# sqeazy/sqeazy

Measured on AMD Instinct MI355X. Metric: encode GB/s (input voxels) for bitswap1->lz4 uint16 volume, higher is better.
Workload: dtype u16

## Files before the change

### sqeazy_amd/csrc/sqy_capi.cpp

```cpp
#include "../../include/sqeazy_amd.h"

#include <hip/hip_runtime.h>

#include <algorithm>
#include <chrono>
#include <climits>
#include <cstdint>
#include <cstdio>
#include <cstdlib>
#include <cstring>
#include <atomic>
#include <condition_variable>
#include <memory>
#include <mutex>
#include <string>
#include <thread>
#include <vector>

#include "sqy_kernels.h"
#include "sqy_lanes.hpp"
#include "sqy_pipeline.hpp"

namespace {

// ... 558 lines not shown
    int produced(const uint8_t* out) { cur = out; return 0; }
    bool is_tail(size_t si) const { return pipe.sink_index >= 0 && (int)si > pipe.sink_index; }
    bool not_3d(const char* scheme) const
    {
        if (dims.size() != 3) std::fprintf(stderr, "[sqeazy::detail::%s::encode] received non-3D shape which is currently unsupported!\n", scheme);
        return dims.size() != 3;
    }
    bool followed_by(size_t si, StageKind k) const { return si + 1 < pipe.stages.size() && pipe.stages[si + 1].kind == k; }
    void stage_shape(size_t si, uint64_t& Z, uint64_t& Y, uint64_t& X) const
    {
        const bool flat = is_tail(si) && cur_len * (uint64_t)cur_elem != len;
        Z = flat ? 1 : dims[0]; Y = flat ? 1 : dims[1]; X = flat ? cur_len : dims[2];
    }

    int take_lanes(std::unique_lock<std::mutex>& lock)
    {
        const long mode = g_opt.stage_lanes.load();
        if (!lanes || mode == 0 || (mode == 2 && !g_opt.transpose_chain_caller_streams.load()) || (stream != nullptr && stream == cx.stream)) return 0;
        int devid = 0;
        if (hipGetDevice(&devid) != hipSuccess || devid < 0 || devid >= kMaxDev) return 0;
        if (!cx.ensure_lane_event()) { std::fprintf(stderr, "[sqeazy]\t no HIP event for the lanes\n"); return 1; }
        const auto deadline = std::chrono::steady_clock::now() + kLaneArrival;
        for (;;) {
            const hipError_t e = hipStreamQuery(stream);
            if (e == hipSuccess) break;
            (void)hipGetLastError();
            if (e != hipErrorNotReady) { std::fprintf(stderr, "[sqeazy]\t HIP error %s while waiting for the caller's stream\n", hipGetErrorString(e)); return 1; }
            if (std::chrono::steady_clock::now() > deadline) { g_opt.lane_backlog_fallbacks += 1; return 0; }
            std::this_thread::yield();
        }
        Lanes& L = g_lanes[devid];
        lock = std::unique_lock<std::mutex>(L.mu);
        const int lane = L.picker.take((int)g_opt.parse_lanes.load());
        if (!L.ensure(lane)) {
            L.picker.give(lane);
            std::fprintf(stderr, "[sqeazy]\t no HIP stream for the lanes\n");
            return 1;
        }
        if (L.picker.total() == 1) {
            const hipError_t r = hipEventRecord(cx.lane_t, L.transpose);
            if (r != hipSuccess || hipEventRecord(cx.lane_p, L.parse[lane]) != hipSuccess) { L.picker.give(lane); SQY_HIP(hipErrorUnknown); }
            lock.unlock();
            const auto answer_by = std::chrono::steady_clock::now() + kLaneAnswer;
            bool alive = false;
            for (;;) {
                const hipError_t et = hipEventQuery(cx.lane_t), ep = et == hipSuccess ? hipEventQuery(cx.lane_p) : et;
                if (et == hipSuccess && ep == hipSuccess) { alive = true; break; }
                (void)hipGetLastError();
                if (std::chrono::steady_clock::now() > answer_by) break;
                std::this_thread::yield();
            }
            lock.lock();
            if (!alive) {
                L.picker.give(lane);
                lock.unlock();
                g_opt.lane_blocked_fallbacks += 1;
                return 0;
            }
        }
        const long seq = g_opt.lane_calls.fetch_add(1);
        if (stamps) { stamps->seq = seq; stamps->lane = lane; stamps->stamp(CallStamps::lanes_taken); }
        lanes->lanes = &L;
        lanes->lane = lane;
        lanes->transpose = L.transpose;
        lanes->parse = L.parse[lane];
        stream = L.transpose;
        return 0;
    }
    int leave_transpose_lane(std::unique_lock<std::mutex>& lock)
    {
        SQY_HIP(hipEventRecord(cx.lane_t, stream));
        lanes->t_done = cx.lane_t;
        lock.unlock();
        stream = lanes->parse;
        SQY_HIP(hipStreamWaitEvent(stream, cx.lane_t, 0));
        return 0;
    }

    int bitswap1(size_t si)
    {
        std::unique_lock<std::mutex> lane_lock;
        uint32_t* ph = nullptr;
        uint64_t gap_chunk = 0;
        if (cur_elem == 2 && followed_by(si, StageKind::lz4)) {
            const sqy::Lz4Params& lz = pipe.stages[si + 1].lz4;
            const uint64_t words = sqy::bitswap1_piece_hash_words(cur, cur, cur_len);
            const uint64_t total = cur_len * 2;
            const uint64_t chunk = lz.bytes_per_chunk(total);
            const bool chunked = chunk <= lz.block_bytes() && !(pipe.nthreads == 1 && total > chunk);
            if (words && chunked && chunk % 1024 == 0 && total > chunk) {
                const uint64_t nch = (total + chunk - 1) / chunk;
                const uint64_t ph_bytes = (words * 4 + 63) & ~(uint64_t)63;
                if (ws->dedupe.ensure(ph_bytes + sqy::lz4_dedupe_work_bytes(nch) + ((nch * 4 + 7) & ~(uint64_t)7) + sqy::lz4_holes_map_bytes(nch, (uint32_t)chunk))) return 1;
                ph = static_cast<uint32_t*>(ws->dedupe.p);
                prep.piece_hash = ph;
                if (dstoffset && si + 2 == pipe.stages.size() && (chunk & (chunk - 1)) == 0) {
                    const uint64_t hdr_max = sqy::header_pack(elem_size, false, dims, pipe.name(), (uint64_t)INT_MAX).size() + 2;
                    uint64_t t0 = hdr_max;
                    while ((reinterpret_cast<uintptr_t>(d_dst) + t0 + 11) & 15) ++t0;
                    if (t0 + nch * (chunk + 15) <= dst_capacity) {
                        gap_chunk = chunk;
                        prep.t0 = t0;
                        prep.in_stride = chunk + 15;
                        prep.inplace = true;
                        if (ws->plan.ensure((nch + 1) * sizeof(uint32_t))) return 1;
                        const uint32_t dstride = sqy::lz4_noise_digest_stride((uint32_t)chunk);
                        if (g_opt.noise_digest.load() && dstride && (cur_len / 8) % chunk == 0 && lz.accel >= 0 &&
                            !ws->digest.ensure(nch * (uint64_t)dstride * sizeof(uint32_t), true)) {
                            prep.digest = static_cast<uint32_t*>(ws->digest.p);
                            prep.digest_stride = dstride;
                        }
                        if (take_lanes(lane_lock)) return 1;
                        SQY_HIP(sqy::launch_lz4_dedupe_clear(static_cast<uint8_t*>(ws->dedupe.p) + ph_bytes, nch, static_cast<uint32_t*>(ws->plan.p), stream));
                        prep.dedupe_cleared = true;
                        if (stamps) stamps->stamp(CallStamps::clear_launched);
                    }
                }
            }
        }
        uint8_t* out = gap_chunk ? static_cast<uint8_t*>(d_dst) + prep.t0 + 11 : next_buf(cur_len * cur_elem);
        if (!out) return 1;
        if (!gap_chunk && ph && (reinterpret_cast<uintptr_t>(out) & 15)) { ph = nullptr; prep.piece_hash = nullptr; }
        const bool on_lanes = lanes && lanes->taken();
        const bool owned = stream != nullptr && stream == cx.stream;
        int devid = 0;
        const bool chain = !on_lanes && g_opt.transpose_chain.load() && (owned || g_opt.transpose_chain_caller_streams.load()) && gap_chunk &&
                           hipGetDevice(&devid) == hipSuccess && devid >= 0 && devid < kMaxDev;
        std::unique_lock<std::mutex> tlock;
        if (chain) {
            if (!cx.t_done && hipEventCreateWithFlags(&cx.t_done, hipEventDisableTiming) != hipSuccess) return 1;
            tlock = std::unique_lock<std::mutex>(g_tchain_mu[devid]);
            const auto now = std::chrono::steady_clock::now();
            if (g_tchain_last[devid] && g_tchain_last[devid] != cx.t_done && now - g_tchain_when[devid] < std::chrono::milliseconds(5))
                SQY_HIP(hipStreamWaitEvent(stream, g_tchain_last[devid], 0));
            g_tchain_when[devid] = now;
        }
        if (cur_elem == 2)
            SQY_TIMED("bitswap1_u16", sqy::launch_bitswap1_u16(reinterpret_cast<const uint16_t*>(cur), reinterpret_cast<uint16_t*>(out), cur_len, stream, ph,
                                                               (uint32_t)gap_chunk, side.p, side.w, side.X, gap_chunk ? prep.digest : nullptr, prep.digest_stride));
        else
            SQY_TIMED("bitswap1_u8", sqy::launch_bitswap1_u8(cur, out, cur_len, stream));
        if (chain) {
            SQY_HIP(hipEventRecord(cx.t_done, stream));
            g_tchain_last[devid] = cx.t_done;
            tlock.unlock();
        }
        if (stamps) stamps->stamp(CallStamps::transpose_launched);
        if (on_lanes && leave_transpose_lane(lane_lock)) return 1;
        side = DiffSide();
        return produced(out);
    }

    int reorder(size_t si, bool zcurve)
    {
        const char* name = zcurve ? "zcurve_reorder" : "raster_reorder";
        if (not_3d(zcurve ? "zcurve" : "reorder")) return 1;
        const Stage& st = pipe.stages[si];
        auto t = st.cfg.find("tile_size");
        const uint64_t ts = t != st.cfg.end() ? (uint64_t)std::atoi(t->second.c_str()) : (zcurve ? 2 : 0);
        uint64_t Z, Y, X;
        stage_shape(si, Z, Y, X);
        if (zcurve ? !sqy::zcurve_geometry_defined(Z, Y, X, ts) : !sqy::raster_geometry_defined(Z, Y, X, ts, cur_elem)) {
            std::fprintf(stderr, "[sqeazy]\t %s: the reference's result is undefined for shape %llux%llux%llu at tile_size=%llu (%s); refused\n", name,
                         (unsigned long long)Z, (unsigned long long)Y, (unsigned long long)X, (unsigned long long)ts,
                         zcurve ? "tile sizes other than 2..128 powers of two, or a tile that does not divide a power-of-two shape"
                                : "remainder in some dimensions only, or a tile wider than one 16-byte block");
            return 1;
        }
        uint8_t* out = next_buf(cur_len * cur_elem);
        if (!out) return 1;
        SQY_TIMED(name, sqy::launch_raster_reorder(cur, out, Z, Y, X, ts, cur_elem, false, stream));
        return produced(out);
    }

    int rmestbkrd()
    {
        const uint64_t portion = sqy::rmestbkrd_face_portion(dims[1] * dims[2], (uint32_t)g_opt.host_l2_bytes.load());
        if (ws->bkrd.ensure(sqy::rmestbkrd_work_bytes(cur_elem))) return 1;
        uint8_t* out = next_buf(cur_len * cur_elem);
        if (!out) return 1;
        SQY_TIMED("rmestbkrd", sqy::launch_rmestbkrd(cur, out, dims[0], dims[1], dims[2], portion, cur_elem, ws->bkrd.p, stream));
        return produced(out);
    }

    int rmbkrd_neighbor5(size_t si)
    {
        const Stage& st = pipe.stages[si];
        const float cut = st.nb_fraction * (float)(125u - 1u);
        uint8_t* out = next_buf(cur_len * cur_elem);
        if (!out) return 1;
        SQY_TIMED("rmbkrd_neighbor5x5x5", sqy::launch_rmbkrd_neighbor5(cur, out, dims[0], dims[1], dims[2], (uint32_t)st.nb_threshold, cut,
                                                                       sqy::neighbor5_z_end(dims[0], dims[2]), cur_elem, stream));
        return produced(out);
    }

    int pass_through() { cur_len *= (uint64_t)cur_elem; cur_elem = 1; return 0; }

    int bitshuffle(size_t si)
    {
        const Stage& st = pipe.stages[si];
        auto b = st.cfg.find("block_size");
        const uint64_t be = sqy::bitshuffle_block_elems(cur_elem, b != st.cfg.end() ? (uint64_t)std::atoi(b->second.c_str()) : 0);
        if (!be) { std::fprintf(stderr, "[sqeazy]\t bitshuffle: block_size must be a multiple of 8\n"); return 1; }
        uint8_t* out = next_buf(cur_len * cur_elem);
        if (!out) return 1;
        SQY_TIMED("bitshuffle", sqy::launch_bitshuffle(cur, out, cur_len, cur_elem, be, false, stream));
        return produced(out);
    }

    template <class Order>
    int shuffle_map(const uint8_t* in, uint64_t units, uint64_t per_unit, bool tail, const char* prof, Order order,
                                std::vector<uint64_t>& map, uint64_t** d_map)
    {
        if (ws->small.ensure(std::max<uint64_t>(units * 16, 4096))) return 1;
        float* d_sums = static_cast<float*>(ws->small.p);
        *d_map = reinterpret_cast<uint64_t*>(static_cast<uint8_t*>(ws->small.p) + ((units * 4 + 15) & ~(uint64_t)15));
        const uint64_t fm_bytes = sqy::frame_metric_scratch_bytes(units, per_unit, cur_elem);
        if (ws->lz4_scratch.ensure(std::max<uint64_t>(fm_bytes, 16))) return 1;
        SQY_TIMED(prof, sqy::launch_frame_metric(in, units, per_unit, cur_elem, d_sums, stream, ws->lz4_scratch.p, fm_bytes, tail));
        std::vector<float> sums(units);
        map.assign(units, 0);
        SQY_HIP(hipMemcpyAsync(sums.data(), d_sums, units * sizeof(float), hipMemcpyDeviceToHost, stream));
// ... 1992 lines not shown
```

### sqeazy_amd/csrc/sqy_kernels.h

```cpp
#ifndef SQY_KERNELS_H_
#define SQY_KERNELS_H_

#include <hip/hip_runtime_api.h>
#include <stdint.h>

namespace sqy {

struct Lz4DedupeArgs {
    const uint64_t* chunk_key = nullptr;
    const uint64_t* tab_key = nullptr;
    const uint32_t* tab_val = nullptr;
    uint32_t tab_mask = 0;
    uint32_t* dup_of = nullptr;
    const uint32_t* piece_hash = nullptr;
    const uint64_t* holes_map = nullptr;
    uint64_t nchunks_full = 0;
    const uint32_t* digest = nullptr;
    uint32_t digest_stride = 0;
};
hipError_t launch_bitswap1_u16(const uint16_t* in, uint16_t* out, uint64_t len, hipStream_t stream, uint32_t* piece_hash = nullptr,
                               uint32_t gap_chunk = 0, const uint16_t* side = nullptr, uint32_t side_w = 0, uint32_t X = 0,
                               uint32_t* digest = nullptr, uint32_t digest_stride = 0);
void set_bitswap1_blocks_per_cu(long n);
uint32_t lz4_noise_digest_stride(uint32_t chunk);
uint64_t bitswap1_piece_hash_words(const void* in, const void* out, uint64_t len);
uint64_t lz4_dedupe_work_bytes(uint64_t nchunks);
hipError_t launch_lz4_dedupe(const uint8_t* in, uint64_t total, uint32_t chunk, const uint32_t* piece_hash, void* work,
                             uint32_t* dup_of, hipStream_t stream, uint64_t in_stride = 0, uint64_t* holes_map = nullptr,
                             bool table_is_clear = false, Lz4DedupeArgs* fused = nullptr);
hipError_t launch_lz4_dedupe_clear(void* work, uint64_t nchunks, uint32_t* zero_word, hipStream_t stream);
uint64_t lz4_holes_map_bytes(uint64_t nchunks, uint32_t chunk);
hipError_t launch_bitswap1_u8(const uint8_t* in, uint8_t* out, uint64_t len, hipStream_t stream);

uint32_t diff3x3x1_side_width(uint64_t Z, uint64_t Y, uint64_t X, int elem_size);
hipError_t launch_diff3x3x1_side(const uint16_t* in, uint16_t* side, uint64_t Z, uint64_t Y, uint64_t X, uint32_t side_w, hipStream_t stream);
hipError_t launch_diff3x3x1(const void* in, void* out, uint64_t Z, uint64_t Y, uint64_t X, int elem_size, hipStream_t stream,
                            bool schar = false);

hipError_t launch_lz4_chunks(const uint8_t* in, uint64_t total, uint32_t chunk, uint8_t* scratch, uint64_t stride,
                             uint32_t* csize, uint64_t nchunks, hipStream_t stream, const uint64_t* frame_map = nullptr,
                             uint64_t frame_bytes = 0, uint32_t* redo = nullptr, const uint32_t* dup_of = nullptr, uint64_t in_stride = 0,
                             uint32_t acceleration = 1,
                             bool redo_is_zero = false,
                             const Lz4DedupeArgs* dedupe = nullptr);
hipError_t launch_lz4_chunks_dense(const uint8_t* in, uint64_t total, uint32_t chunk, uint8_t* scratch, uint64_t stride,
                                   uint32_t* csize, uint32_t* redo, uint32_t redo_count, hipStream_t stream,
                                   const uint64_t* frame_map = nullptr, uint64_t frame_bytes = 0, uint64_t in_stride = 0);
struct Lz4Block {
    uint64_t start;
    uint32_t n;
    uint32_t flags;
    int64_t low_in, low_dict;
};
hipError_t launch_lz4_linked(const uint8_t* in, const Lz4Block* blocks, const uint32_t* frame_first, uint64_t nframes,
                             uint32_t max_block, uint8_t* scratch, uint64_t stride, uint32_t* csize, hipStream_t stream, uint32_t acceleration = 1);
struct Lz4SpecArgs {
    const uint32_t* wave_first = nullptr;
    const uint32_t* wave_last = nullptr;
    uint32_t* tables = nullptr;
    uint32_t mode = 0;
};
constexpr uint64_t kLz4SpecTableWords = 2 * 4096;
hipError_t launch_lz4_linked_spec(const uint8_t* in, const Lz4Block* blocks, const Lz4SpecArgs& spec, uint64_t nwaves,
                                  uint32_t max_block, uint8_t* scratch, uint64_t stride, uint32_t* csize, hipStream_t stream, uint32_t acceleration = 1);
hipError_t launch_lz4_linked_verify(const Lz4Block* blocks, uint64_t nblocks, const uint32_t* tables, uint32_t max_block, uint32_t* ok, hipStream_t stream);
hipError_t launch_lz4_frame_scan(const uint32_t* csize, uint64_t nchunks, uint64_t total, uint32_t chunk,
                                 uint64_t* frame_off, hipStream_t stream, const Lz4Block* blocks = nullptr,
                                 const uint32_t* dup_of = nullptr, uint64_t* tail_info = nullptr,
                                 const uint32_t* guard = nullptr, uint8_t* body0 = nullptr, uint64_t in_stride = 0, uint32_t bd_byte = 0,
                                 uint32_t hc_byte = 0);
hipError_t launch_lz4_inplace_tail_fused(uint8_t* out, uint64_t t0, uint64_t in_stride, uint64_t total, uint32_t chunk, uint64_t nchunks,
                                         const uint8_t* scratch, uint64_t stride, const uint32_t* csize, uint64_t* frame_off, const uint32_t* dup_of,
                                         uint64_t* tail_info, uint32_t bd_byte, uint32_t hc_byte, const char* hdr_prefix, uint32_t prefix_len,
                                         const char* hdr_suffix, uint32_t suffix_len, uint32_t elem_size, const uint32_t* guard, uint64_t* record,
                                         hipStream_t stream);
hipError_t launch_lz4_inplace_tail(uint8_t* out, uint64_t t0, uint64_t in_stride, uint64_t total, uint32_t chunk, uint64_t nchunks,
                                   uint8_t* scratch, uint64_t stride, const uint32_t* csize, const uint64_t* frame_off, const uint32_t* dup_of,
                                   const uint64_t* tail_info, uint32_t bd_byte, uint32_t hc_byte, const char* hdr_prefix, uint32_t prefix_len,
                                   const char* hdr_suffix, uint32_t suffix_len, uint32_t elem_size, const uint32_t* guard, uint64_t* record,
                                   hipStream_t stream);
constexpr uint32_t kLz4InplaceHeaderTextMax = 3000;
hipError_t launch_lz4_tail_marks(uint8_t* body0, uint64_t in_stride, uint64_t total, uint32_t chunk, uint64_t nchunks, uint32_t bd_byte,
                                 uint32_t hc_byte, const uint64_t* tail_info, hipStream_t stream);
hipError_t launch_lz4_stash_raw(const uint8_t* body0, uint64_t in_stride, uint64_t total, uint32_t chunk, uint8_t* scratch, uint64_t stride,
                                const uint32_t* csize, const uint32_t* dup_of, uint64_t nhead, hipStream_t stream);
hipError_t launch_lz4_frame_gather(const uint8_t* in, uint64_t total, uint32_t chunk, const uint8_t* scratch, uint64_t stride,
                                   const uint32_t* csize, const uint64_t* frame_off, uint8_t* out, uint32_t bd_byte,
                                   uint32_t hc_byte, uint64_t nchunks, hipStream_t stream, const uint64_t* frame_map = nullptr,
                                   uint64_t frame_bytes = 0, const Lz4Block* blocks = nullptr, const uint32_t* dup_of = nullptr,
                                   uint64_t in_stride = 0, bool raw_from_scratch = false);

uint64_t rmestbkrd_work_bytes(int elem_size);
hipError_t launch_rmestbkrd(const void* in, void* out, uint64_t Z, uint64_t Y, uint64_t X, uint64_t portion, int elem_size, void* work,
                            hipStream_t stream);
hipError_t launch_rmbkrd_neighbor5(const void* in, void* out, uint64_t Z, uint64_t Y, uint64_t X, uint32_t threshold, float cut,
                                   uint64_t z_end, int elem_size, hipStream_t stream);
hipError_t launch_histogram_u16(const uint16_t* in, uint64_t len, uint32_t* histo, hipStream_t stream);
hipError_t launch_quantiser_apply_u16(const uint16_t* in, uint8_t* out, uint64_t len, const uint8_t* lut, hipStream_t stream);
hipError_t launch_quantiser_apply_bitswap1_u8(const uint16_t* in, uint8_t* out, uint64_t len, const uint8_t* lut, hipStream_t stream);

hipError_t launch_raster_reorder(const void* in, void* out, uint64_t Z, uint64_t Y, uint64_t X, uint64_t tile_size, int elem_size,
                                 bool decode, hipStream_t stream);

hipError_t launch_bitshuffle(const void* in, void* out, uint64_t n_elems, int elem_size, uint64_t block_elems, bool decode, hipStream_t stream);

hipError_t launch_frame_metric(const void* in, uint64_t Z, uint64_t per_frame, int elem_size, float* metric, hipStream_t stream,
                               void* scratch = nullptr, uint64_t scratch_bytes = 0, bool schar = false);
uint64_t frame_metric_scratch_bytes(uint64_t Z, uint64_t per_frame, int elem_size);
hipError_t launch_frame_gather(const void* in, void* out, uint64_t Z, uint64_t frame_bytes, const uint64_t* map, hipStream_t stream);

hipError_t launch_lz4_frame_index(const uint8_t* in, uint64_t n, void* blk, uint32_t* frame_first, uint64_t max_blocks,
                                  uint32_t* counts , hipStream_t stream);
uint64_t lz4_frame_rank_scratch_bytes(uint64_t expected_frames);
// ... 58 lines not shown
```

### sqeazy_amd/csrc/sqy_kernels.hip

```cpp
#include <hip/hip_runtime.h>
#include <atomic>
#include <mutex>
#include <stdint.h>
#include <cstring>
#include <type_traits>

#include "sqy_kernels.h"

namespace sqy {

struct __attribute__((packed)) pk_u16 { uint16_t v; };
struct __attribute__((packed)) pk_u32 { uint32_t v; };
struct __attribute__((packed)) pk_u64 { uint64_t v; };
struct __attribute__((packed)) pk_u128 { uint32_t x, y, z, w; };

__device__ __forceinline__ uint32_t ld_u32(const uint8_t* p) { return reinterpret_cast<const pk_u32*>(p)->v; }
__device__ __forceinline__ uint64_t ld_u64(const uint8_t* p) { return reinterpret_cast<const pk_u64*>(p)->v; }
__device__ __forceinline__ uint4 ld_u128(const uint8_t* p)
{
    const pk_u128 t = *reinterpret_cast<const pk_u128*>(p);
    return make_uint4(t.x, t.y, t.z, t.w);
}
__device__ __forceinline__ void st_u32(uint8_t* p, uint32_t v) { reinterpret_cast<pk_u32*>(p)->v = v; }
__device__ __forceinline__ void st_u128(uint8_t* p, uint4 v)
// ... 24 lines not shown
    const volatile SQY_LDS al4_u64* q = reinterpret_cast<const volatile SQY_LDS al4_u64*>(p);
    const al4_u64 a = { q[0].x, q[0].y }, b = { q[1].x, q[1].y };
    return make_uint4(a.x, a.y, b.x, b.y);
}
__device__ __forceinline__ uint2 lds_ld_2dw(const lds_u8* p)
{
    const volatile SQY_LDS al4_u64* q = reinterpret_cast<const volatile SQY_LDS al4_u64*>(p);
    return make_uint2(q->x, q->y);
}
__device__ __forceinline__ uint32_t lds_ld_u32_via_aligned(const lds_u8* base, uint32_t at)
{
    const uint2 d = lds_ld_2dw(base + (at & ~3u));
    return __builtin_amdgcn_alignbyte(d.y, d.x, at & 3u);
}
__device__ __forceinline__ uint32_t glb_ld_u8(glb_u8* p) { return *p; }
__device__ __forceinline__ uint4 ld_u128_agent(const uint8_t* p)
{
    v4u v;
    asm volatile("global_load_dwordx4 %0, %1, off sc1\n\ts_waitcnt vmcnt(0)" : "=v"(v) : "v"(p) : "memory");
    return make_uint4(v.x, v.y, v.z, v.w);
}
__device__ __forceinline__ uint32_t glb_ld_u32(glb_u8* p) { return reinterpret_cast<SQY_GLB const pk_u32*>(p)->v; }
__device__ __forceinline__ uint64_t glb_ld_u64(glb_u8* p) { return reinterpret_cast<SQY_GLB const pk_u64*>(p)->v; }
__device__ __forceinline__ uint4 glb_ld_u128(glb_u8* p)
{
    SQY_GLB const pk_u128* q = reinterpret_cast<SQY_GLB const pk_u128*>(p);
    return make_uint4(q->x, q->y, q->z, q->w);
}

__device__ __forceinline__ void wave_lds_sync()
{
    __builtin_amdgcn_fence(__ATOMIC_RELEASE, "wavefront");
    __builtin_amdgcn_wave_barrier();
    __builtin_amdgcn_fence(__ATOMIC_ACQUIRE, "wavefront");
}
__device__ __forceinline__ uint32_t sgpr(uint32_t v) { return __builtin_amdgcn_readfirstlane(v); }
__device__ __forceinline__ uint32_t lane_read(uint32_t v, uint32_t l) { return __builtin_amdgcn_readlane(v, l); }
__device__ __forceinline__ uint32_t lane_write(uint32_t v, uint32_t x, uint32_t l)
{
    uint32_t km;
    asm("s_mov_b32 %1, m0\n\ts_mov_b32 m0, %3\n\tv_writelane_b32 %0, %2, m0\n\ts_mov_b32 m0, %1" : "+v"(v), "=&s"(km) : "s"(x), "s"(l));
    return v;
}
__device__ __forceinline__ uint64_t ballot(bool p) { return __builtin_amdgcn_ballot_w64(p); }
__device__ __forceinline__ uint32_t ctz64(uint64_t m) { return (uint32_t)__builtin_ctzll(m); }

constexpr int BSW_TILE_VOX = 8192;

__device__ __forceinline__ void transpose16x16_pairs(uint32_t r[16])
{
#pragma unroll
    for (int i = 0; i < 8; ++i) {
        const uint32_t a = r[i], b = r[i + 8];
        r[i] = __builtin_amdgcn_perm(b, a, 0x06020400u);
        r[i + 8] = __builtin_amdgcn_perm(b, a, 0x07030501u);
    }
#pragma unroll
    for (int blk = 0; blk < 16; blk += 8) {
#pragma unroll
        for (int i = 0; i < 4; ++i) {
            const uint32_t a = r[blk + i], b = r[blk + i + 4];
            r[blk + i] = (a & 0x0f0f0f0fu) | ((b << 4) & 0xf0f0f0f0u);
            r[blk + i + 4] = ((a >> 4) & 0x0f0f0f0fu) | (b & 0xf0f0f0f0u);
        }
    }
#pragma unroll
    for (int blk = 0; blk < 16; blk += 4) {
#pragma unroll
        for (int i = 0; i < 2; ++i) {
            const uint32_t a = r[blk + i], b = r[blk + i + 2];
            r[blk + i] = (a & 0x33333333u) | ((b << 2) & 0xccccccccu);
            r[blk + i + 2] = ((a >> 2) & 0x33333333u) | (b & 0xccccccccu);
        }
    }
#pragma unroll
    for (int blk = 0; blk < 16; blk += 2) {
        const uint32_t a = r[blk], b = r[blk + 1];
        r[blk] = (a & 0x55555555u) | ((b << 1) & 0xaaaaaaaau);
        r[blk + 1] = ((a >> 1) & 0x55555555u) | (b & 0xaaaaaaaau);
    }
}

__device__ __forceinline__ uint32_t lz4_hash5_32(uint32_t lo, uint32_t byte4);
template <bool GAP>
__global__ __launch_bounds__(256)
void bitswap1_u16_regs(const uint16_t* __restrict__ in, uint16_t* __restrict__ out, uint64_t n_tiles, uint64_t seg_words,
                       uint32_t* __restrict__ piece_hash, uint32_t gap_shift, const uint16_t* __restrict__ side, uint32_t side_w, uint32_t X,
                       uint32_t* __restrict__ digest, uint32_t digest_stride)
{
    const int lane = threadIdx.x & 63;
    const uint32_t wpb = blockDim.x >> 6;
    const uint64_t wave_global = (uint64_t)blockIdx.x * wpb + (uint32_t)__builtin_amdgcn_readfirstlane((int)(threadIdx.x >> 6));
    const uint64_t wave_stride = (uint64_t)gridDim.x * wpb;
    for (uint64_t tile = wave_global; tile < n_tiles; tile += wave_stride) {
        const v4u* src = reinterpret_cast<const v4u*>(in + tile * BSW_TILE_VOX) + lane * 16;
        if (side) {
            const uint64_t i0 = tile * BSW_TILE_VOX + (uint64_t)lane * 128u;
            const uint64_t row = i0 / X;
            const uint32_t x0 = (uint32_t)(i0 - row * X);
            if (x0 < side_w) src = reinterpret_cast<const v4u*>(side + row * side_w + x0);
        }
        v4u v[16];
#pragma unroll
        for (int j = 0; j < 16; ++j) v[j] = src[j];
        uint32_t pl[16][4];
#pragma unroll
        for (int q = 0; q < 4; ++q) {
            const v4u a0 = v[4 * q], a1 = v[4 * q + 1], b0 = v[4 * q + 2], b1 = v[4 * q + 3];
            const uint32_t ga[8] = {a0.x, a0.y, a0.z, a0.w, a1.x, a1.y, a1.z, a1.w};
            const uint32_t gb[8] = {b0.x, b0.y, b0.z, b0.w, b1.x, b1.y, b1.z, b1.w};
            uint32_t r[16];
#pragma unroll
            for (int k = 0; k < 8; ++k) {
                r[15 - 2 * k] = __builtin_amdgcn_perm(gb[k], ga[k], 0x05040100u);
                r[14 - 2 * k] = __builtin_amdgcn_perm(gb[k], ga[k], 0x07060302u);
            }
            transpose16x16_pairs(r);
#pragma unroll
            for (int b = 0; b < 16; ++b) pl[b][q] = r[b];
        }
        uint32_t dg = 0;
        if (GAP && digest) {
            const uint32_t x = (((uint32_t)tile << 10) & ((1u << gap_shift) - 1u)) + (uint32_t)lane * 16u;
            if (x + 16u > 7667u) {
                const uint32_t xx = x > 7667u ? x : 7667u;
                uint32_t st = (uint32_t)((1.0f + __builtin_sqrtf(1.0f + (float)(xx - 2u) * 0.125f)) * 0.5f);
                if (2u + 32u * (st + 1u) * st <= xx) ++st;
                if (2u + 32u * st * (st - 1u) > xx) --st;
                const uint32_t Bs = 2u + 32u * st * (st - 1u), num = xx - Bs;
                uint32_t kk = (uint32_t)((float)num / (float)st);
                if (kk * st > num) --kk;
                if ((kk + 1u) * st <= num) ++kk;
                if (kk * st != num) ++kk;
                const uint32_t cand = Bs + kk * st, u = 64u * st - 62u + kk;
                if (cand < x + 16u && u >= 961u && u - 961u < digest_stride) dg = 0x80000000u | ((u - 961u) << 4) | (cand - x);
            }
        }
        const uint32_t dg_tsh = 31u - gap_shift;
        const uint32_t pm = 2u * (uint32_t)lane + 1u;
#pragma unroll
        for (int b = 0; b < 16; ++b) {
            uint32_t vx = pl[b][0], vy = pl[b][1], vz = pl[b][2], vw = pl[b][3];
            asm volatile("" : "+v"(vx), "+v"(vy), "+v"(vz), "+v"(vw) :: "memory");
            const v4u val = {vx, vy, vz, vw};
            const uint64_t nzm = ballot((val.x | val.y | val.z | val.w) != 0u);
            if (piece_hash) {
                uint32_t a = val.x * 0x9E3779B1u + val.y * 0x85EBCA77u + val.z * 0xC2B2AE3Du + val.w * 0x27D4EB2Fu;
                a = (a ^ (a >> 15)) * pm;
                const bool row_nz = ((nzm >> (lane & 48)) & 0xffffull) != 0ull;
                a += __builtin_amdgcn_update_dpp(0u, a, 0x111, 0xf, 0xf, false);
                a += __builtin_amdgcn_update_dpp(0u, a, 0x112, 0xf, 0xf, false);
                a += __builtin_amdgcn_update_dpp(0u, a, 0x114, 0xf, 0xf, false);
                a += __builtin_amdgcn_update_dpp(0u, a, 0x118, 0xf, 0xf, false);
                const uint64_t piece = ((uint64_t)(15 - b) * seg_words * 2u + tile * 1024u) >> 10;
                if ((lane & 15) == 15) piece_hash[piece * 4u + (uint32_t)(lane >> 4)] = row_nz ? (a | 1u) : 0u;
            }
            if (GAP) {
                if (nzm == 0ull) continue;
                const uint64_t B = (uint64_t)(15 - b) * seg_words * 2u + tile * 1024u;
                if (digest) {
                    const uint32_t nx = (uint32_t)__builtin_amdgcn_update_dpp(0, (int)val.x, 0x130, 0xf, 0xf, true);
                    const uint32_t dg_off = dg & 15u, dg_q = dg_off >> 2, dg_r = dg_off & 3u;
                    const uint32_t d0 = dg_q == 0u ? val.x : dg_q == 1u ? val.y : dg_q == 2u ? val.z : val.w;
                    const uint32_t d1 = dg_q == 0u ? val.y : dg_q == 1u ? val.z : dg_q == 2u ? val.w : nx;
                    const uint32_t lo = __builtin_amdgcn_alignbyte(d1, d0, dg_r);
                    const uint32_t b5 = d1 >> (8u * dg_r);
                    uint32_t e = (lz4_hash5_32(lo, b5) << 17) | ((lo * 2654435761u) >> (32u - dg_tsh));
                    if (lane == 63 && dg_off > 11u) e = 0xffffffffu;
                    const uint64_t drow = (B >> gap_shift) * (uint64_t)digest_stride * 4u;
                    const uint32_t drow_lo = (uint32_t)__builtin_amdgcn_readfirstlane((int)(uint32_t)drow);
                    const uint32_t drow_hi = (uint32_t)__builtin_amdgcn_readfirstlane((int)(uint32_t)(drow >> 32));
                    uint8_t* const dbase = reinterpret_cast<uint8_t*>(digest) + (((uint64_t)drow_hi << 32) | drow_lo);
                    if ((int32_t)dg < 0) *reinterpret_cast<uint32_t*>(dbase + ((dg >> 2) & 0x1ffffffcu)) = e;
                }
                const uint64_t kq = B >> gap_shift;
#ifdef SQY_EXP_GAP_BYTES
                const uint64_t off = B + kq * SQY_EXP_GAP_BYTES;
#else
                const uint64_t off = B + (kq << 4) - kq;
#endif
                const uint32_t off_lo = (uint32_t)__builtin_amdgcn_readfirstlane((int)(uint32_t)off);
                const uint32_t off_hi = (uint32_t)__builtin_amdgcn_readfirstlane((int)(uint32_t)(off >> 32));
                uint8_t* dst = reinterpret_cast<uint8_t*>(out) + (((uint64_t)off_hi << 32) | off_lo);
                __builtin_nontemporal_store((v4u_any)val, reinterpret_cast<v4u_any*>(dst + (uint32_t)lane * 16u));
            } else {
                v4u* dst = reinterpret_cast<v4u*>(out + (uint64_t)(15 - b) * seg_words + tile * (BSW_TILE_VOX / 16));
                __builtin_nontemporal_store(val, dst + lane);
            }
        }
    }
}

__global__ __launch_bounds__(64)
void lz4_dedupe_key_kernel(const uint32_t* __restrict__ piece_hash, uint32_t pieces_per_chunk, uint64_t nchunks_full,
                           uint64_t* __restrict__ chunk_key, uint64_t* __restrict__ tab_key, uint32_t* __restrict__ tab_val, uint32_t tab_mask,
                           uint64_t* __restrict__ holes_map, uint32_t pieces_last)
{
    const uint64_t k = blockIdx.x;
    const int lane = threadIdx.x;
    const uint32_t* ph = piece_hash + k * pieces_per_chunk * 4u;
    const uint32_t np = k < nchunks_full ? pieces_per_chunk : pieces_last;
    uint64_t* hm = holes_map ? holes_map + k * (1u + (pieces_per_chunk + 63u) / 64u) : nullptr;
    uint32_t h1 = 0, h2 = 0, any = 0, nzero = 0;
    for (uint32_t base = 0; base < np; base += 64) {
        const uint32_t i = base + (uint32_t)lane;
        uint4 q = make_uint4(1u, 0u, 0u, 0u);
        if (i < np) q = *reinterpret_cast<const uint4*>(ph + i * 4u);
        any |= i < np ? (q.x | q.y | q.z | q.w) : 0u;
        const uint32_t s_ = i < np ? q.x + q.y + q.z + q.w : 0u;
        h1 += s_ * ((2u * i + 1u) * 0x9E3779B1u);
        h2 += ((s_ << 13) | (s_ >> 19)) * ((2u * i + 3u) * 0x85EBCA77u);
        if (hm) {
            const uint64_t zm = ballot((q.x | q.y | q.z | q.w) == 0u);
            nzero += (uint32_t)__builtin_popcountll(zm);
            if (lane == 0) hm[1u + base / 64u] = zm;
        }
    }
    if (hm && lane == 0) hm[0] = nzero;
    if (k >= nchunks_full) return;
// ... 4656 lines not shown
                                   uint64_t hx, uint64_t zlim, int single, uint64_t r0, uint64_t r1)
{
    const uint64_t frame = Y * X;
    const uint64_t r = r0 + (uint64_t)blockIdx.x * blockDim.x + threadIdx.x;
    if (r >= r1) return;
    const uint64_t idx = z * frame + r;
    T v = in[idx];
    if (z >= 1 && diff_touched(idx, length, Y, X, hx, zlim, single != 0)) {
        const T* p = out + idx - frame;
        T sum = 0;
        sum = (T)(sum + p[-(int64_t)X - 1]); sum = (T)(sum + p[-(int64_t)X]); sum = (T)(sum + p[-(int64_t)X + 1]);
        sum = (T)(sum + p[-1]);              sum = (T)(sum + p[0]);           sum = (T)(sum + p[1]);
        sum = (T)(sum + p[X - 1]);           sum = (T)(sum + p[X]);           sum = (T)(sum + p[X + 1]);
        v = (T)((uint32_t)(int32_t)(ST)v + (SCHAR ? (uint32_t)(uint16_t)(int16_t)(int8_t)sum / 9u : (uint32_t)sum / 9u));
    }
    out[idx] = v;
}



__global__ __launch_bounds__(256)
void quantiser_decode_kernel(const uint8_t* __restrict__ in, uint16_t* __restrict__ out, uint64_t len, const uint16_t* __restrict__ lut)
{
    __shared__ uint16_t sl[256];
    sl[threadIdx.x] = lut[threadIdx.x];
    __syncthreads();
    const uint64_t nvec = ((reinterpret_cast<uintptr_t>(in) & 7) == 0 && (reinterpret_cast<uintptr_t>(out) & 15) == 0) ? len / 8 : 0;
    for (uint64_t v = (uint64_t)blockIdx.x * 256 + threadIdx.x; v < nvec; v += (uint64_t)gridDim.x * 256) {
        const uint2 x = reinterpret_cast<const uint2*>(in)[v];
        uint4 y;
        y.x = (uint32_t)sl[x.x & 0xffu] | ((uint32_t)sl[(x.x >> 8) & 0xffu] << 16);
        y.y = (uint32_t)sl[(x.x >> 16) & 0xffu] | ((uint32_t)sl[x.x >> 24] << 16);
        y.z = (uint32_t)sl[x.y & 0xffu] | ((uint32_t)sl[(x.y >> 8) & 0xffu] << 16);
        y.w = (uint32_t)sl[(x.y >> 16) & 0xffu] | ((uint32_t)sl[x.y >> 24] << 16);
        reinterpret_cast<uint4*>(out)[v] = y;
    }
    for (uint64_t i = nvec * 8 + (uint64_t)blockIdx.x * 256 + threadIdx.x; i < len; i += (uint64_t)gridDim.x * 256) out[i] = sl[in[i]];
}

__global__ __launch_bounds__(256)
void frame_scatter_kernel(const uint8_t* __restrict__ in, uint8_t* __restrict__ out, uint64_t frame_bytes,
                          const uint64_t* __restrict__ map, uint32_t blocks_per_frame)
{
    const uint64_t f = blockIdx.x / blocks_per_frame;
    const uint32_t part = blockIdx.x % blocks_per_frame;
    const uint8_t* s = in + f * frame_bytes;
    const uint64_t to = map[f];
    if (to == ~0ull) return;
    uint8_t* d = out + to * frame_bytes;
    const uint64_t nvec = frame_bytes / 16;
    if (((reinterpret_cast<uintptr_t>(s) | reinterpret_cast<uintptr_t>(d)) & 15) == 0) {
        const uint64_t step = (uint64_t)blocks_per_frame * 256;
        for (uint64_t v0 = (uint64_t)part * 256 + threadIdx.x; v0 < nvec; v0 += 4 * step) {
            uint4 t[4];
#pragma unroll
            for (uint32_t j = 0; j < 4; ++j) if (v0 + j * step < nvec) t[j] = reinterpret_cast<const uint4*>(s)[v0 + j * step];
#pragma unroll
            for (uint32_t j = 0; j < 4; ++j) if (v0 + j * step < nvec) reinterpret_cast<uint4*>(d)[v0 + j * step] = t[j];
        }
        if (part == 0)
            for (uint64_t i = nvec * 16 + threadIdx.x; i < frame_bytes; i += 256) d[i] = s[i];
    } else {
        for (uint64_t i = (uint64_t)part * 256 + threadIdx.x; i < frame_bytes; i += (uint64_t)blocks_per_frame * 256) d[i] = s[i];
    }
}

static inline int num_cus()
{
    static int cus = 0;
    if (!cus) {
        int dev = 0;
        (void)hipGetDevice(&dev);
        hipDeviceProp_t p;
        if (hipGetDeviceProperties(&p, dev) == hipSuccess) cus = p.multiProcessorCount;
        if (cus <= 0) cus = 256;
    }
    return cus;
}

std::atomic<long> g_bsw_blocks_per_cu{32};
void set_bitswap1_blocks_per_cu(long n) { g_bsw_blocks_per_cu.store(n); }

hipError_t launch_bitswap1_u16(const uint16_t* in, uint16_t* out, uint64_t len, hipStream_t stream, uint32_t* piece_hash, uint32_t gap_chunk,
                               const uint16_t* side, uint32_t side_w, uint32_t X, uint32_t* digest, uint32_t digest_stride)
{
    if (len == 0) return hipSuccess;
    if (side && (X == 0 || X % 128u != 0 || side_w % 128u != 0 || side_w > X || len % X != 0 || (reinterpret_cast<uintptr_t>(side) & 15) ||
                 len % BSW_TILE_VOX != 0 || (reinterpret_cast<uintptr_t>(in) & 15) || (!gap_chunk && (reinterpret_cast<uintptr_t>(out) & 15))))
        return hipErrorInvalidValue;
    if (gap_chunk) {
        if (len % BSW_TILE_VOX != 0 || (reinterpret_cast<uintptr_t>(in) & 15) || gap_chunk < 1024u || (gap_chunk & (gap_chunk - 1u)) || !piece_hash)
            return hipErrorInvalidValue;
        const uint64_t n_tiles = len / BSW_TILE_VOX, want = (n_tiles + 1) / 2, cap = (uint64_t)num_cus() * (g_bsw_blocks_per_cu.load() > 0 ? (uint64_t)g_bsw_blocks_per_cu.load() : 32u);
        if (digest && ((len / 8) % gap_chunk != 0 || gap_chunk < 16384u || digest_stride == 0)) return hipErrorInvalidValue;
        hipLaunchKernelGGL(bitswap1_u16_regs<true>, dim3((unsigned)(want < cap ? want : cap)), dim3(128), 0, stream, in, out, n_tiles, len / 16,
                           piece_hash, (uint32_t)__builtin_ctz(gap_chunk), side, side_w, X, digest, digest_stride);
        return hipGetLastError();
    }
    const uint64_t seg_words = len / 16;
    uint64_t n_tiles = 0;
    const bool aligned = (seg_words % 8 == 0) && ((reinterpret_cast<uintptr_t>(in) & 15) == 0) &&
                         ((reinterpret_cast<uintptr_t>(out) & 15) == 0);
    if (aligned) n_tiles = (seg_words * 16) / BSW_TILE_VOX;
    if (piece_hash && n_tiles * BSW_TILE_VOX != len) return hipErrorInvalidValue;
    if (n_tiles) {
        const uint64_t want = (n_tiles + 1) / 2;
        const uint64_t cap = (uint64_t)num_cus() * 32;
        const unsigned grid = (unsigned)(want < cap ? want : cap);
        hipLaunchKernelGGL(bitswap1_u16_regs<false>, dim3(grid), dim3(128), 0, stream, in, out, n_tiles, seg_words, piece_hash, 0u, side, side_w, X,
                           (uint32_t*)nullptr, 0u);
    }
    const uint64_t first_word = n_tiles * (BSW_TILE_VOX / 16);
    const uint64_t rest_words = seg_words - first_word;
    const uint64_t tail = len - seg_words * 16;
    if (rest_words || tail) {
        uint64_t blocks = (rest_words + 255) / 256;
        if (blocks == 0) blocks = 1;
        hipLaunchKernelGGL(bitswap1_u16_generic, dim3((unsigned)blocks), dim3(256), 0, stream, in, out, len, first_word, seg_words);
    }
    return hipGetLastError();
}

uint32_t lz4_noise_digest_stride(uint32_t chunk)
{
    if (chunk < 16384u || (chunk & (chunk - 1u))) return 0;
    uint64_t p = 1, st = 1, nb = 64, probes = 0;
    for (;;) {
        ++probes;
        const uint64_t p2 = p + st;
        st = nb >> 6; ++nb;
        if (p2 > (uint64_t)chunk - 12 + 1) break;
        p = p2;
    }
    if (probes <= 961) return 0;
    return (uint32_t)(((probes - 960) + 63) & ~(uint64_t)63);
}

uint64_t bitswap1_piece_hash_words(const void* in, const void* out, uint64_t len)
{
    if (len == 0 || len % BSW_TILE_VOX != 0) return 0;
    if ((reinterpret_cast<uintptr_t>(in) & 15) || (reinterpret_cast<uintptr_t>(out) & 15)) return 0;
    return (len / BSW_TILE_VOX) * 16 * 4;
}

__global__ __launch_bounds__(256)
void lz4_dedupe_clear_kernel(uint64_t* __restrict__ tab_key, uint32_t* __restrict__ tab_val, uint32_t tab, uint32_t* __restrict__ zero_word)
{
    const uint32_t i = blockIdx.x * 256u + threadIdx.x;
    if (i < tab) { tab_key[i] = 0ull; tab_val[i] = 0xffffffffu; }
    if (i == 0 && zero_word) *zero_word = 0u;
}

hipError_t launch_lz4_dedupe_clear(void* work, uint64_t nchunks, uint32_t* zero_word, hipStream_t stream)
{
    if (nchunks == 0) return hipSuccess;
    uint32_t tab = 64;
    while (tab < 2 * nchunks) tab <<= 1;
    uint64_t* chunk_key = static_cast<uint64_t*>(work);
    uint64_t* tab_key = chunk_key + nchunks;
    uint32_t* tab_val = reinterpret_cast<uint32_t*>(tab_key + tab);
    hipLaunchKernelGGL(lz4_dedupe_clear_kernel, dim3((tab + 255u) / 256u), dim3(256), 0, stream, tab_key, tab_val, tab, zero_word);
    return hipGetLastError();
}

hipError_t launch_lz4_dedupe(const uint8_t* in, uint64_t total, uint32_t chunk, const uint32_t* piece_hash, void* work,
                             uint32_t* dup_of, hipStream_t stream, uint64_t in_stride, uint64_t* holes_map, bool table_is_clear,
                             Lz4DedupeArgs* fused)
{
    const uint64_t nchunks = (total + chunk - 1) / chunk, nfull = total / chunk;
    if (nchunks == 0) return hipSuccess;
    if (in_stride == 0) in_stride = chunk;
    if (chunk % 1024 != 0) return hipErrorInvalidValue;
    uint32_t tab = 64;
    while (tab < 2 * nchunks) tab <<= 1;
    uint64_t* chunk_key = static_cast<uint64_t*>(work);
    uint64_t* tab_key = chunk_key + nchunks;
    uint32_t* tab_val = reinterpret_cast<uint32_t*>(tab_key + tab);
    hipError_t e = hipSuccess;
    if (!table_is_clear) {
        e = hipMemsetAsync(tab_key, 0, (size_t)tab * 8, stream);
        if (e != hipSuccess) return e;
        e = hipMemsetAsync(tab_val, 0xff, (size_t)tab * 4, stream);
        if (e != hipSuccess) return e;
    }
    if (holes_map && total % 1024u != 0) return hipErrorInvalidValue;
    const uint64_t nkey = holes_map ? nchunks : nfull;
    if (nkey)
        hipLaunchKernelGGL(lz4_dedupe_key_kernel, dim3((unsigned)nkey), dim3(64), 0, stream, piece_hash, chunk / 1024u, nfull, chunk_key, tab_key,
                           tab_val, tab - 1u, holes_map, (uint32_t)((total - nfull * chunk) >> 10));
    if (fused) {
        fused->chunk_key = chunk_key; fused->tab_key = tab_key; fused->tab_val = tab_val; fused->tab_mask = tab - 1u; fused->dup_of = dup_of;
        fused->piece_hash = piece_hash; fused->holes_map = holes_map; fused->nchunks_full = nfull;
        return hipGetLastError();
    }
    hipLaunchKernelGGL(lz4_dedupe_verify_kernel, dim3((unsigned)nchunks), dim3(DEDUPE_THREADS), 0, stream, in, chunk, in_stride, nfull, nchunks, chunk_key,
                       tab_key, tab_val, tab - 1u, dup_of, piece_hash, holes_map, total);
    return hipGetLastError();
}

uint64_t lz4_holes_map_bytes(uint64_t nchunks, uint32_t chunk)
{
    return nchunks * (1u + ((uint64_t)(chunk >> 10) + 63u) / 64u) * 8u;
}

uint64_t lz4_dedupe_work_bytes(uint64_t nchunks)
{
    uint64_t tab = 64;
    while (tab < 2 * nchunks) tab <<= 1;
    return nchunks * 8 + tab * 8 + tab * 4 + 64;
}

hipError_t launch_quantiser_apply_bitswap1_u8(const uint16_t* in, uint8_t* out, uint64_t len, const uint8_t* lut, hipStream_t stream)
{
    if (len == 0) return hipSuccess;
    if (reinterpret_cast<uintptr_t>(in) & 15) return hipErrorInvalidValue;
    uint64_t blocks = (len / 8 + 256 * 16 - 1) / (256 * 16);
    const uint64_t cap = (uint64_t)num_cus() * 2;
    if (blocks > cap) blocks = cap;
    if (blocks == 0) blocks = 1;
    hipLaunchKernelGGL(quantiser_apply_bitswap1_u8_kernel, dim3((unsigned)blocks), dim3(256), 65536, stream, in, out, len, lut);
    return hipGetLastError();
}

hipError_t launch_bitswap1_u8(const uint8_t* in, uint8_t* out, uint64_t len, hipStream_t stream)
{
    if (len == 0) return hipSuccess;
    const uint64_t seg = len / 8;
    uint64_t blocks = (seg + 127) / 128;
    if (blocks == 0) blocks = 1;
    hipLaunchKernelGGL(bitswap1_u8_generic, dim3((unsigned)blocks), dim3(128), 0, stream, in, out, len, seg);
    return hipGetLastError();
}

uint32_t diff3x3x1_side_width(uint64_t Z, uint64_t Y, uint64_t X, int elem_size)
{
    const uint64_t length = Z * Y * X;
    if (length == 0 || elem_size != 2 || X % 128 != 0 || length % BSW_TILE_VOX != 0) return 0;
    const uint64_t zlim = X < Z ? X : Z;
    const uint64_t noff = (zlim >= 1 ? (zlim - 1) : 0) * (Y >= 2 ? (Y - 2) : 0);
    if (noff == 1) return 0;
    const uint64_t hx = Z >= 2 ? Z - 2 : 0;
    if (!(hx + 2 <= X && Y <= 65535 && Z <= 65535 && X <= 0xffffffffull)) return 0;
    const uint64_t w = ((1 + hx) + 127) / 128 * 128;
    return w < X ? (uint32_t)w : 0;
}
// ... 1337 lines not shown
```

Measured before the change: 2055.

## Fuse dedupe table clear into bitswap kernel and template side path

Removes the separate dedupe hash-table clear kernel launch. The bitswap1 u16 kernel now zeroes the table with a grid-stride loop before transposing, which saves one launch and one dependency on the stream. The side-buffer branch becomes a template parameter, so the common path carries no per-tile side check. An experimental load pattern using permlane swaps is added but disabled by default.

Measured after the change: 2011. 2.1% lower.

```diff
diff --git a/sqeazy_amd/csrc/sqy_capi.cpp b/sqeazy_amd/csrc/sqy_capi.cpp
--- a/sqeazy_amd/csrc/sqy_capi.cpp
+++ b/sqeazy_amd/csrc/sqy_capi.cpp
@@ -664,6 +664,7 @@
         std::unique_lock<std::mutex> lane_lock;
         uint32_t* ph = nullptr;
         uint64_t gap_chunk = 0;
+        sqy::Lz4DedupeClear clear;
         if (cur_elem == 2 && followed_by(si, StageKind::lz4)) {
             const sqy::Lz4Params& lz = pipe.stages[si + 1].lz4;
             const uint64_t words = sqy::bitswap1_piece_hash_words(cur, cur, cur_len);
@@ -693,7 +694,7 @@
                             prep.digest_stride = dstride;
                         }
                         if (take_lanes(lane_lock)) return 1;
-                        SQY_HIP(sqy::launch_lz4_dedupe_clear(static_cast<uint8_t*>(ws->dedupe.p) + ph_bytes, nch, static_cast<uint32_t*>(ws->plan.p), stream));
+                        clear = sqy::lz4_dedupe_clear_args(static_cast<uint8_t*>(ws->dedupe.p) + ph_bytes, nch, static_cast<uint32_t*>(ws->plan.p));
                         prep.dedupe_cleared = true;
                         if (stamps) stamps->stamp(CallStamps::clear_launched);
                     }
@@ -719,7 +720,7 @@
         }
         if (cur_elem == 2)
             SQY_TIMED("bitswap1_u16", sqy::launch_bitswap1_u16(reinterpret_cast<const uint16_t*>(cur), reinterpret_cast<uint16_t*>(out), cur_len, stream, ph,
-                                                               (uint32_t)gap_chunk, side.p, side.w, side.X, gap_chunk ? prep.digest : nullptr, prep.digest_stride));
+                                                               (uint32_t)gap_chunk, side.p, side.w, side.X, gap_chunk ? prep.digest : nullptr, prep.digest_stride, clear));
         else
             SQY_TIMED("bitswap1_u8", sqy::launch_bitswap1_u8(cur, out, cur_len, stream));
         if (chain) {
diff --git a/sqeazy_amd/csrc/sqy_kernels.h b/sqeazy_amd/csrc/sqy_kernels.h
--- a/sqeazy_amd/csrc/sqy_kernels.h
+++ b/sqeazy_amd/csrc/sqy_kernels.h
@@ -18,9 +18,15 @@
     const uint32_t* digest = nullptr;
     uint32_t digest_stride = 0;
 };
+struct Lz4DedupeClear {
+    uint64_t* tab_key = nullptr;
+    uint32_t* tab_val = nullptr;
+    uint32_t tab = 0;
+    uint32_t* zero_word = nullptr;
+};
 hipError_t launch_bitswap1_u16(const uint16_t* in, uint16_t* out, uint64_t len, hipStream_t stream, uint32_t* piece_hash = nullptr,
                                uint32_t gap_chunk = 0, const uint16_t* side = nullptr, uint32_t side_w = 0, uint32_t X = 0,
-                               uint32_t* digest = nullptr, uint32_t digest_stride = 0);
+                               uint32_t* digest = nullptr, uint32_t digest_stride = 0, Lz4DedupeClear clear = Lz4DedupeClear());
 void set_bitswap1_blocks_per_cu(long n);
 uint32_t lz4_noise_digest_stride(uint32_t chunk);
 uint64_t bitswap1_piece_hash_words(const void* in, const void* out, uint64_t len);
@@ -28,7 +34,7 @@
 hipError_t launch_lz4_dedupe(const uint8_t* in, uint64_t total, uint32_t chunk, const uint32_t* piece_hash, void* work,
                              uint32_t* dup_of, hipStream_t stream, uint64_t in_stride = 0, uint64_t* holes_map = nullptr,
                              bool table_is_clear = false, Lz4DedupeArgs* fused = nullptr);
-hipError_t launch_lz4_dedupe_clear(void* work, uint64_t nchunks, uint32_t* zero_word, hipStream_t stream);
+Lz4DedupeClear lz4_dedupe_clear_args(void* work, uint64_t nchunks, uint32_t* zero_word);
 uint64_t lz4_holes_map_bytes(uint64_t nchunks, uint32_t chunk);
 hipError_t launch_bitswap1_u8(const uint8_t* in, uint8_t* out, uint64_t len, hipStream_t stream);
 
diff --git a/sqeazy_amd/csrc/sqy_kernels.hip b/sqeazy_amd/csrc/sqy_kernels.hip
--- a/sqeazy_amd/csrc/sqy_kernels.hip
+++ b/sqeazy_amd/csrc/sqy_kernels.hip
@@ -130,42 +130,60 @@
 }
 
 __device__ __forceinline__ uint32_t lz4_hash5_32(uint32_t lo, uint32_t byte4);
-template <bool GAP>
+#ifndef SQY_EXP_BSW_LOADS
+#define SQY_EXP_BSW_LOADS 0
+#endif
+__device__ __forceinline__ void rows4x4_swap(v4u& a0, v4u& a1, v4u& a2, v4u& a3)
+{
+#pragma unroll
+    for (int d = 0; d < 4; ++d) {
+        const auto p02 = __builtin_amdgcn_permlane32_swap(a0[d], a2[d], false, false);
+        const auto p13 = __builtin_amdgcn_permlane32_swap(a1[d], a3[d], false, false);
+        const auto q01 = __builtin_amdgcn_permlane16_swap(p02[0], p13[0], false, false);
+        const auto q23 = __builtin_amdgcn_permlane16_swap(p02[1], p13[1], false, false);
+        a0[d] = q01[0]; a1[d] = q01[1]; a2[d] = q23[0]; a3[d] = q23[1];
+    }
+}
+template <bool GAP, bool SIDE>
 __global__ __launch_bounds__(256)
 void bitswap1_u16_regs(const uint16_t* __restrict__ in, uint16_t* __restrict__ out, uint64_t n_tiles, uint64_t seg_words,
                        uint32_t* __restrict__ piece_hash, uint32_t gap_shift, const uint16_t* __restrict__ side, uint32_t side_w, uint32_t X,
-                       uint32_t* __restrict__ digest, uint32_t digest_stride)
+                       uint32_t* __restrict__ digest, uint32_t digest_stride,
+                       uint64_t* __restrict__ tab_key, uint32_t* __restrict__ tab_val, uint32_t tab, uint32_t* __restrict__ zero_word)
 {
     const int lane = threadIdx.x & 63;
+    if (tab_key) {
+        const uint32_t i0 = blockIdx.x * blockDim.x + threadIdx.x;
+        if (i0 < tab) {
+            for (uint32_t i = i0; i < tab; i += gridDim.x * blockDim.x) { tab_key[i] = 0ull; tab_val[i] = 0xffffffffu; }
+        }
+        if (i0 == 0 && zero_word) *zero_word = 0u;
+    }
     const uint32_t wpb = blockDim.x >> 6;
     const uint64_t wave_global = (uint64_t)blockIdx.x * wpb + (uint32_t)__builtin_amdgcn_readfirstlane((int)(threadIdx.x >> 6));
     const uint64_t wave_stride = (uint64_t)gridDim.x * wpb;
     for (uint64_t tile = wave_global; tile < n_tiles; tile += wave_stride) {
-        const v4u* src = reinterpret_cast<const v4u*>(in + tile * BSW_TILE_VOX) + lane * 16;
-        if (side) {
-            const uint64_t i0 = tile * BSW_TILE_VOX + (uint64_t)lane * 128u;
-            const uint64_t row = i0 / X;
-            const uint32_t x0 = (uint32_t)(i0 - row * X);
-            if (x0 < side_w) src = reinterpret_cast<const v4u*>(side + row * side_w + x0);
-        }
+        constexpr bool RUNS = !SIDE && SQY_EXP_BSW_LOADS != 0;
         v4u v[16];
-#pragma unroll
-        for (int j = 0; j < 16; ++j) v[j] = src[j];
-        uint32_t pl[16][4];
-#pragma unroll
-        for (int q = 0; q < 4; ++q) {
-            const v4u a0 = v[4 * q], a1 = v[4 * q + 1], b0 = v[4 * q + 2], b1 = v[4 * q + 3];
-            const uint32_t ga[8] = {a0.x, a0.y, a0.z, a0.w, a1.x, a1.y, a1.z, a1.w};
-            const uint32_t gb[8] = {b0.x, b0.y, b0.z, b0.w, b1.x, b1.y, b1.z, b1.w};
-            uint32_t r[16];
-#pragma unroll
-            for (int k = 0; k < 8; ++k) {
-                r[15 - 2 * k] = __builtin_amdgcn_perm(gb[k], ga[k], 0x05040100u);
-                r[14 - 2 * k] = __builtin_amdgcn_perm(gb[k], ga[k], 0x07060302u);
-            }
-            transpose16x16_pairs(r);
-#pragma unroll
-            for (int b = 0; b < 16; ++b) pl[b][q] = r[b];
+        if (RUNS) {
+            const v4u* src = reinterpret_cast<const v4u*>(in + tile * BSW_TILE_VOX) + (lane & 15) * 16 + (lane >> 4);
+#pragma unroll
+            for (int kl = 0; kl < 4; ++kl) {
+#pragma unroll
+                for (int kh = 0; kh < 4; ++kh)
+                    v[4 * kl + kh] = SQY_EXP_BSW_LOADS == 2 ? __builtin_nontemporal_load(src + 256 * kh + 4 * kl) : src[256 * kh + 4 * kl];
+                __builtin_amdgcn_sched_barrier(0);
+            }
+        } else {
+            const v4u* src = reinterpret_cast<const v4u*>(in + tile * BSW_TILE_VOX) + lane * 16;
+            if (SIDE) {
+                const uint64_t i0 = tile * BSW_TILE_VOX + (uint64_t)lane * 128u;
+                const uint64_t row = i0 / X;
+                const uint32_t x0 = (uint32_t)(i0 - row * X);
+                if (x0 < side_w) src = reinterpret_cast<const v4u*>(side + row * side_w + x0);
+            }
+#pragma unroll
+            for (int j = 0; j < 16; ++j) v[j] = src[j];
         }
         uint32_t dg = 0;
         if (GAP && digest) {
@@ -183,6 +201,26 @@
                 const uint32_t cand = Bs + kk * st, u = 64u * st - 62u + kk;
                 if (cand < x + 16u && u >= 961u && u - 961u < digest_stride) dg = 0x80000000u | ((u - 961u) << 4) | (cand - x);
             }
+        }
+        uint32_t pl[16][4];
+#pragma unroll
+        for (int q = 0; q < 4; ++q) {
+            if (RUNS) {
+                __builtin_amdgcn_sched_barrier(0);
+                rows4x4_swap(v[4 * q], v[4 * q + 1], v[4 * q + 2], v[4 * q + 3]);
+            }
+            const v4u a0 = v[4 * q], a1 = v[4 * q + 1], b0 = v[4 * q + 2], b1 = v[4 * q + 3];
+            const uint32_t ga[8] = {a0.x, a0.y, a0.z, a0.w, a1.x, a1.y, a1.z, a1.w};
+            const uint32_t gb[8] = {b0.x, b0.y, b0.z, b0.w, b1.x, b1.y, b1.z, b1.w};
+            uint32_t r[16];
+#pragma unroll
+            for (int k = 0; k < 8; ++k) {
+                r[15 - 2 * k] = __builtin_amdgcn_perm(gb[k], ga[k], 0x05040100u);
+                r[14 - 2 * k] = __builtin_amdgcn_perm(gb[k], ga[k], 0x07060302u);
+            }
+            transpose16x16_pairs(r);
+#pragma unroll
+            for (int b = 0; b < 16; ++b) pl[b][q] = r[b];
         }
         const uint32_t dg_tsh = 31u - gap_shift;
         const uint32_t pm = 2u * (uint32_t)lane + 1u;
@@ -5005,7 +5043,7 @@
 void set_bitswap1_blocks_per_cu(long n) { g_bsw_blocks_per_cu.store(n); }
 
 hipError_t launch_bitswap1_u16(const uint16_t* in, uint16_t* out, uint64_t len, hipStream_t stream, uint32_t* piece_hash, uint32_t gap_chunk,
-                               const uint16_t* side, uint32_t side_w, uint32_t X, uint32_t* digest, uint32_t digest_stride)
+                               const uint16_t* side, uint32_t side_w, uint32_t X, uint32_t* digest, uint32_t digest_stride, Lz4DedupeClear clear)
 {
     if (len == 0) return hipSuccess;
     if (side && (X == 0 || X % 128u != 0 || side_w % 128u != 0 || side_w > X || len % X != 0 || (reinterpret_cast<uintptr_t>(side) & 15) ||
@@ -5016,8 +5054,13 @@
             return hipErrorInvalidValue;
         const uint64_t n_tiles = len / BSW_TILE_VOX, want = (n_tiles + 1) / 2, cap = (uint64_t)num_cus() * (g_bsw_blocks_per_cu.load() > 0 ? (uint64_t)g_bsw_blocks_per_cu.load() : 32u);
         if (digest && ((len / 8) % gap_chunk != 0 || gap_chunk < 16384u || digest_stride == 0)) return hipErrorInvalidValue;
-        hipLaunchKernelGGL(bitswap1_u16_regs<true>, dim3((unsigned)(want < cap ? want : cap)), dim3(128), 0, stream, in, out, n_tiles, len / 16,
-                           piece_hash, (uint32_t)__builtin_ctz(gap_chunk), side, side_w, X, digest, digest_stride);
+        const dim3 grid((unsigned)(want < cap ? want : cap));
+        if (side)
+            hipLaunchKernelGGL((bitswap1_u16_regs<true, true>), grid, dim3(128), 0, stream, in, out, n_tiles, len / 16, piece_hash,
+                               (uint32_t)__builtin_ctz(gap_chunk), side, side_w, X, digest, digest_stride, clear.tab_key, clear.tab_val, clear.tab, clear.zero_word);
+        else
+            hipLaunchKernelGGL((bitswap1_u16_regs<true, false>), grid, dim3(128), 0, stream, in, out, n_tiles, len / 16, piece_hash,
+                               (uint32_t)__builtin_ctz(gap_chunk), side, side_w, X, digest, digest_stride, clear.tab_key, clear.tab_val, clear.tab, clear.zero_word);
         return hipGetLastError();
     }
     const uint64_t seg_words = len / 16;
@@ -5030,8 +5073,12 @@
         const uint64_t want = (n_tiles + 1) / 2;
         const uint64_t cap = (uint64_t)num_cus() * 32;
         const unsigned grid = (unsigned)(want < cap ? want : cap);
-        hipLaunchKernelGGL(bitswap1_u16_regs<false>, dim3(grid), dim3(128), 0, stream, in, out, n_tiles, seg_words, piece_hash, 0u, side, side_w, X,
-                           (uint32_t*)nullptr, 0u);
+        if (side)
+            hipLaunchKernelGGL((bitswap1_u16_regs<false, true>), dim3(grid), dim3(128), 0, stream, in, out, n_tiles, seg_words, piece_hash, 0u, side, side_w, X,
+                               (uint32_t*)nullptr, 0u, clear.tab_key, clear.tab_val, clear.tab, clear.zero_word);
+        else
+            hipLaunchKernelGGL((bitswap1_u16_regs<false, false>), dim3(grid), dim3(128), 0, stream, in, out, n_tiles, seg_words, piece_hash, 0u, side, side_w, X,
+                               (uint32_t*)nullptr, 0u, clear.tab_key, clear.tab_val, clear.tab, clear.zero_word);
     }
     const uint64_t first_word = n_tiles * (BSW_TILE_VOX / 16);
     const uint64_t rest_words = seg_words - first_word;
@@ -5066,24 +5113,18 @@
     return (len / BSW_TILE_VOX) * 16 * 4;
 }
 
-__global__ __launch_bounds__(256)
-void lz4_dedupe_clear_kernel(uint64_t* __restrict__ tab_key, uint32_t* __restrict__ tab_val, uint32_t tab, uint32_t* __restrict__ zero_word)
-{
-    const uint32_t i = blockIdx.x * 256u + threadIdx.x;
-    if (i < tab) { tab_key[i] = 0ull; tab_val[i] = 0xffffffffu; }
-    if (i == 0 && zero_word) *zero_word = 0u;
-}
-
-hipError_t launch_lz4_dedupe_clear(void* work, uint64_t nchunks, uint32_t* zero_word, hipStream_t stream)
-{
-    if (nchunks == 0) return hipSuccess;
+Lz4DedupeClear lz4_dedupe_clear_args(void* work, uint64_t nchunks, uint32_t* zero_word)
+{
+    Lz4DedupeClear c;
+    if (nchunks == 0) return c;
     uint32_t tab = 64;
     while (tab < 2 * nchunks) tab <<= 1;
     uint64_t* chunk_key = static_cast<uint64_t*>(work);
-    uint64_t* tab_key = chunk_key + nchunks;
-    uint32_t* tab_val = reinterpret_cast<uint32_t*>(tab_key + tab);
-    hipLaunchKernelGGL(lz4_dedupe_clear_kernel, dim3((tab + 255u) / 256u), dim3(256), 0, stream, tab_key, tab_val, tab, zero_word);
-    return hipGetLastError();
+    c.tab_key = chunk_key + nchunks;
+    c.tab_val = reinterpret_cast<uint32_t*>(c.tab_key + tab);
+    c.tab = tab;
+    c.zero_word = zero_word;
+    return c;
 }
 
 hipError_t launch_lz4_dedupe(const uint8_t* in, uint64_t total, uint32_t chunk, const uint32_t* piece_hash, void* work,
```
